# kubernetes-sigs/karpenter

Hardware: AMD Instinct MI355X
Metric: pods scheduled/sec (Solve()) (higher is better)
Workload: dtype int64

## Files before the change

karpenter_amd/csrc/fast_engine.h:

```cpp
#pragma once
#include <type_traits>
#include "kernels.h"
#include "pdq_emul.h"

namespace ks {

constexpr int kFastRows = 4;
constexpr uint32_t kFastFree = 0xFFFFFFFFu;
constexpr uint32_t kFastLastBit = 0x80000000u;
constexpr int kFastEnt = 1024;
constexpr int kFastPool = 256;
constexpr int kFastMaxPareto = 16;
constexpr int kFastMaxVar = 12;
constexpr uint64_t kFastExtBit = 1ull << 63;
constexpr int kFastVarBits = 56;

struct FastClaim { uint64_t vmask; int32_t req[4]; };
template <int R> struct FastRec { uint64_t vmask; int32_t req[4]; uint64_t acc[R]; };
struct FastSlot { uint64_t cvmask; uint64_t dmask; int32_t size[4]; uint32_t tmplok; uint32_t kdef; };
struct FastEnt { uint64_t vmask; int32_t cap[4]; uint32_t info; uint32_t pad; };

struct FastPlan {
  int total_bytes, cap;
  int off_state, off_key, off_ord, off_snap, off_ent, off_pool, off_slot, off_misc, off_hot;
  int global_state;
  int rows;
  int helper;
};

struct FastMisc {
  uint64_t tvmask[32];
  uint32_t tdef[32];
  uint64_t fmask[kFastMaxVar];
  uint8_t vkey[kFastMaxVar], voff[kFastMaxVar], vwidth[kFastMaxVar];
  uint16_t vword[kFastMaxVar];
  uint64_t its[kMaxItWords], rem[kMaxItWords], cand[kMaxItWords];
  uint64_t acc[kFastRows];
};

struct FastVar { int nv; uint8_t vkey[kFastMaxVar], voff[kFastMaxVar], vwidth[kFastMaxVar]; uint16_t vword[kFastMaxVar]; };

struct FastNodes {
  uint32_t n_left;
  uint32_t n_placed;
  uint32_t limit_hit;
  uint32_t variant;
  uint32_t bail;
  unsigned long long n_ref;
  unsigned long long n_tests;
};

struct FastWork {
  FastVar* var;
  FastSlot* cls;
  uint32_t* c_hostseq;
  uint16_t* c_ent;
  FastClaim* c_state;
  uint32_t* c_npods;
  uint64_t* ent_its;
  uint32_t* q_class;
  uint32_t* q_claim;
  uint32_t* q_cnt;
  uint16_t* o_key;
  uint16_t* o_ord;
  uint16_t* o_snap;
  uint64_t* c_rec;
  uint32_t* cls_first;
  uint32_t* cls_last;
  uint32_t* max_active;
  FastNodes* nodes;
  uint32_t* nd_pod;
  const uint64_t* nd_dead0;
  FastPlan plan;
  int enabled;
};

typedef uint64_t __attribute__((may_alias)) u64_alias;
template <class T>
KS_FN T lds_get(const KS_LDS T* p) {
  static_assert(sizeof(T) % 8 == 0, "lds_get: 8-byte multiples");
  T out;
  u64_alias* o = (u64_alias*)&out;
  const KS_LDS u64_alias* s = (const KS_LDS u64_alias*)p;
#pragma unroll
  for (int i = 0; i < (int)(sizeof(T) / 8); ++i) o[i] = s[i];
  return out;
}
template <class T>
KS_FN void lds_put(KS_LDS T* p, const T& v) {
  static_assert(sizeof(T) % 8 == 0, "lds_put: 8-byte multiples");
  const u64_alias* o = (const u64_alias*)&v;
  KS_LDS u64_alias* s = (KS_LDS u64_alias*)p;
#pragma unroll
  for (int i = 0; i < (int)(sizeof(T) / 8); ++i) s[i] = o[i];
}

// ... 143 lines not shown
KS_FN uint32_t fast_umin_s(uint32_t a, uint32_t b) {
#if KS_DEVICE
  uint32_t r;
  asm("s_min_u32 %0, %1, %2" : "=s"(r) : "s"(a), "s"(b) : "scc");
  return r;
#else
  return a < b ? a : b;
#endif
}
KS_FN bool fast_sampled(int n, int p) {
  const unsigned q = (unsigned)n >> 2, u = (unsigned)p;
  return u - (q - 1) <= 2u || u - (2 * q - 1) <= 2u || u - (3 * q - 1) <= 2u;
}

struct FastMail {
  uint32_t word[2];
  uint32_t done;
  uint32_t gen;
  uint32_t quit;
  int32_t miss_x[2];
  uint32_t helper;
  uint32_t simd[4];
};
#if KS_DEVICE
KS_FN uint32_t mail_load(const KS_LDS uint32_t* p) { return *(const volatile KS_LDS uint32_t*)p; }
KS_FN void mail_store(KS_LDS uint32_t* p, uint32_t v) { *(volatile KS_LDS uint32_t*)p = v; }
#else
KS_FN uint32_t mail_load(const uint32_t* p) { return *p; }
KS_FN void mail_store(uint32_t* p, uint32_t v) { *p = v; }
#endif

struct FastHot {
  alignas(16) FastMail mail;
  int base, bi, bn, n, np, max_steps, steps, status;
  int pend_a, pend_x, pend_new, ev_arg;
  uint32_t pend_mv;
  int rf_x;
  int rf_x2;
  unsigned long long n_steps, n_tests, n_ref, hot_cycles;
  unsigned long long tsec[8];
  unsigned long long hw[4];
  const uint32_t* q_class; const volatile int* cancel; uint32_t* q_claim; uint32_t* q_cnt;
  uint32_t cur[kFastRows][64];
  uint32_t scls[kFastRows][64];
  uint32_t bcls[64], oclaim[64], ocnt[64], nxt_cls[64];
};

template <class W, int GS, int R>
struct FastCold {
  const ProblemView* Pk;
  const Workspace* Sk;
  const FastWork* Fk;
  typedef typename FastMem<GS, R>::o16 o16;
  ClaimOrder<W, o16, false> order;
  typename FastMem<GS, R>::s16 snap;
  typename FastMem<GS, R>::States cst;
  KS_LDS FastEnt* ent;
  KS_LDS int32_t* pool;
  KS_LDS FastSlot* aslot;
  KS_LDS FastMisc* Mp;
  KS_LDS FastHot* hs;
  int n_claims = 0, nv = 0, n_ent = 0, n_pool = 0, n_evict = 0;
  uint32_t host_seq = 0, active_templates = 0;
  int bail_code = 0;
  int lo_ = 0, hi_ = -1;
  unsigned long long n_ref_extra = 0, n_cold_tests = 0;

  KS_DEV void init(const ProblemView* p, const Workspace* s, const FastWork* f, char* lds) {
    Pk = p; Sk = s; Fk = f;
    const FastPlan& pl = f->plan;
    Mp = (KS_LDS FastMisc*)(lds + pl.off_misc);
    hs = (KS_LDS FastHot*)(lds + pl.off_hot);
    if constexpr (GS >= 1) cst.p = (FastRec<R>*)f->c_rec; else cst.p = (KS_LDS FastRec<R>*)(lds + pl.off_state);
    typedef typename FastMem<GS, R>::s16 s16;
    if constexpr (GS >= 2) { order.key = (o16)f->o_key; order.ord = (o16)f->o_ord; }
    else { order.key = (o16)(lds + pl.off_key); order.ord = (o16)(lds + pl.off_ord); }
    if constexpr (GS >= 1) snap = (s16)f->o_snap; else snap = (s16)(lds + pl.off_snap);
    order.pos = nullptr;
    ent = (KS_LDS FastEnt*)(lds + pl.off_ent);
    pool = (KS_LDS int32_t*)(lds + pl.off_pool);
    aslot = (KS_LDS FastSlot*)(lds + pl.off_slot);
  }

  KS_COLD int create_entry(uint64_t vm) {
    vm = W::uniform(vm);
    const ProblemView& P = *Pk; const Workspace& S = *Sk; const FastWork& F = *Fk;
    const int t = (int)(vm >> 56);
    const int iw = P.it_words, n_its = P.n_its, nr = P.n_res;
    const Dict& d = P.dict;
    const ProblemView& Pv = P;
    KS_LDS FastMisc& Mm = *Mp;
    const uint64_t* tits = S.t_its + (size_t)t * iw;
    KS_LDS uint64_t* its = Mp->its;
    const int nvv = nv;
    W::for_n(iw, [&](int w) {
      uint64_t acc = tits[w];
      for (int j = 0; j < nvv; ++j) {
        const int k = Mm.vkey[j];
        if (!((Pv.it_keys >> k) & 1u)) continue;
        if ((vm >> (Mm.voff[j] + Mm.vwidth[j])) & 1) continue;
        uint64_t field = (vm >> Mm.voff[j]) & (Mm.fmask[j] >> Mm.voff[j]);
        uint64_t r = Pv.key_undef[(size_t)k * iw + w];
        const size_t base = (size_t)Mm.vword[j] * 64;
        while (field) { const int b = ctz64(field); field &= field - 1; r |= Pv.kv_has[(base + b) * iw + w]; }
        acc &= r;
      }
      its[w] = acc;
    });
    uint32_t zones = (1u << P.n_zones) - 1, cts = (1u << P.n_cts) - 1;
    {
      const uint64_t* tm = P.tmpl_reqs.mask + (size_t)t * d.req_words;
      const uint32_t tdef = Mp->tdef[t];
      if (d.key_zone >= 0 && ((tdef >> d.key_zone) & 1u)) zones &= (uint32_t)tm[d.key_word_off[d.key_zone]];
      if (d.key_ct >= 0 && ((tdef >> d.key_ct) & 1u)) cts &= (uint32_t)tm[d.key_word_off[d.key_ct]];
      for (int j = 0; j < nv; ++j) {
        const uint32_t field = (uint32_t)((vm >> Mp->voff[j]) & (Mp->fmask[j] >> Mp->voff[j]));
        if (Mp->vkey[j] == d.key_zone) zones &= field;
        if (Mp->vkey[j] == d.key_ct) cts &= field;
      }
    }
    uint64_t cells = 0;
    for (uint32_t z = zones; z; z &= z - 1) cells |= (uint64_t)cts << (__builtin_ctz(z) * 4);
    for (int j = 0; j < iw; ++j) {
      const uint64_t in = its[j];
      const uint64_t okm = in ? W::ballot([&](int l) { const int it = j * 64 + l; return it < n_its && ((in >> l) & 1) && (Pv.it_off_avail[it] & cells) != 0; }) : 0ull;
      W::store(&its[j], okm);
    }
    W::sync();
    if (n_ent * 5 >= kFastEnt * 4) return -1;
    uint32_t h = fast_hash(vm);
    while (ent[h].info & 1u) h = (h + 1) & (kFastEnt - 1);
    uint64_t* eits = F.ent_its + (size_t)h * iw;
    W::for_n(iw, [&](int w) { eits[w] = its[w]; });
    KS_LDS uint64_t* rem = Mp->rem; KS_LDS uint64_t* cand = Mp->cand;
    W::for_n(iw, [&](int w) { rem[w] = its[w]; });
    int count = 0;
    const int poff = n_pool;
    int32_t f0 = -1, f1 = -1, f2 = -1, f3 = -1;
    const int64_t* eff = eff_alloc(P, t);
    for (;;) {
      const uint64_t any = W::reduce_or(iw, [&](int w) { return (uint64_t)rem[w]; });
      if (!any) break;
      W::for_n(iw, [&](int w) { cand[w] = rem[w]; });
      int64_t v0 = 0x3FFFFFFF, v1 = 0x3FFFFFFF, v2 = 0x3FFFFFFF, v3 = 0x3FFFFFFF;
      for (int r = 0; r < nr; ++r) {
        const int64_t* al = eff + (size_t)r * n_its;
        const int64_t mx = W::reduce_max_i64(iw * 64, [&](int it) { return (it < n_its && ((cand[it >> 6] >> (it & 63)) & 1)) ? al[it] : INT64_MIN; });
        if (r == 0) v0 = mx; else if (r == 1) v1 = mx; else if (r == 2) v2 = mx; else v3 = mx;
        for (int j = 0; j < iw; ++j) {
          const uint64_t in = cand[j];
          const uint64_t eq = in ? W::ballot([&](int l) { const int it = j * 64 + l; return it < n_its && ((in >> l) & 1) && al[it] == mx; }) : 0ull;
          W::store(&cand[j], eq);
        }
        W::sync();
      }
      if (count == 0) { f0 = (int32_t)v0; f1 = (int32_t)v1; f2 = (int32_t)v2; f3 = (int32_t)v3; }
      else {
        if (count > kFastMaxPareto || n_pool >= kFastPool) return -1;
        if (W::leader()) { pool[n_pool * 4 + 0] = (int32_t)v0; pool[n_pool * 4 + 1] = (int32_t)v1; pool[n_pool * 4 + 2] = (int32_t)v2; pool[n_pool * 4 + 3] = (int32_t)v3; }
        n_pool++;
      }
      count++;
      for (int j = 0; j < iw; ++j) {
        const uint64_t in = rem[j];
        const uint64_t dom = in ? W::ballot([&](int l) {
          const int it = j * 64 + l;
          if (it >= n_its || !((in >> l) & 1)) return false;
          bool le = eff[it] <= v0;
          if (nr > 1) le = le && eff[(size_t)n_its + it] <= v1;
          if (nr > 2) le = le && eff[(size_t)2 * n_its + it] <= v2;
          if (nr > 3) le = le && eff[(size_t)3 * n_its + it] <= v3;
          return le;
        }) : 0ull;
        W::store(&rem[j], in & ~dom);
      }
      W::sync();
    }
    if (W::leader()) {
      FastEnt e;
      e.vmask = count > 1 ? (vm | kFastExtBit) : vm; e.cap[0] = f0; e.cap[1] = f1; e.cap[2] = f2; e.cap[3] = f3;
      e.info = 1u | ((uint32_t)(count > 1 ? count - 1 : 0) << 8) | ((uint32_t)poff << 16);
      e.pad = 0;
      lds_put(&ent[h], e);
    }
    n_ent++;
    W::sync();
    return (int)h;
  }

  KS_COLD int setup(bool topo = false) {
    const ProblemView& P = *Pk; const Workspace& S = *Sk; const FastWork& F = *Fk;
    const Dict& d = P.dict;
    const int nk = d.n_keys, iw = P.it_words, nr = P.n_res, n_its = P.n_its, nc = P.n_classes, T = P.n_templates;
    const ProblemView& Pv = P;
    if (!(topo ? P.plain_topo : (P.plain || (F.nodes && P.plain_nodes))) || P.n_rows != P.n_pods || nr > 4 || T > 32 || iw > kMaxItWords) return 1;
    if (W::reduce_or(T, [&](int t) { return (uint64_t)(Pv.tmpl_reqs.complement[t] | (Pv.tmpl_reqs.has_gte ? Pv.tmpl_reqs.has_gte[t] : 0) | (Pv.tmpl_reqs.has_lte ? Pv.tmpl_reqs.has_lte[t] : 0)); })) return 3;
    if (W::reduce_or(nc, [&](int c) { return (uint64_t)Pv.cls_reqs.complement[c]; })) return 4;
    uint32_t vk = (uint32_t)W::reduce_or(nc, [&](int c) { return (uint64_t)Pv.cls_reqs.defined[c]; });
    if (topo) vk |= (uint32_t)W::reduce_or(P.topo.n_groups, [&](int g) { return Pv.topo.key[g] >= 0 ? (uint64_t)1 << Pv.topo.key[g] : (uint64_t)0; });
    if (d.key_hostname >= 0 && ((vk >> d.key_hostname) & 1u)) return 5;
    if (d.key_it >= 0 && ((vk >> d.key_it) & 1u)) return 5;
    int bits = 0;
    nv = 0;
    for (int k = 0; k < nk; ++k) {
      if (!((vk >> k) & 1u)) continue;
      if (d.key_word_off[k + 1] - d.key_word_off[k] != 1 || nv >= kFastMaxVar) return 6;
      const uint64_t valid = d.value_valid[d.key_word_off[k]];
      const int width = valid ? 64 - __builtin_clzll(valid) : 1;
      if (bits + width + 1 > kFastVarBits) return 6;
      if (W::leader()) {
        Mp->vkey[nv] = (uint8_t)k; Mp->voff[nv] = (uint8_t)bits; Mp->vwidth[nv] = (uint8_t)width; Mp->vword[nv] = (uint16_t)d.key_word_off[k];
        Mp->fmask[nv] = ((1ull << width) - 1) << bits;
      }
      bits += width + 1;
      nv++;
    }
    W::sync();
    if (W::leader()) {
      FastVar fv;
      fv.nv = nv;
      for (int j = 0; j < kFastMaxVar; ++j) { fv.vkey[j] = Mp->vkey[j]; fv.voff[j] = Mp->voff[j]; fv.vwidth[j] = Mp->vwidth[j]; fv.vword[j] = Mp->vword[j]; }
      *F.var = fv;
    }
    W::sync();
    if (W::reduce_or(nr * n_its, [&](int i) { const int64_t a = Pv.it_alloc[i]; return (uint64_t)((a >= (1ll << 30) || a <= -(1ll << 30)) ? 1 : 0); })) return 7;
    for (int t = 0; t < T; ++t) {
      if (!((P.tmpl_ov >> t) & 1u)) continue;
      const int64_t* eff = eff_alloc(P, t);
      if (W::reduce_or(nr * n_its, [&](int i) { const int64_t a = eff[i]; return (uint64_t)((a >= (1ll << 30) || a <= -(1ll << 30)) ? 1 : 0); })) return 7;
    }
    if (W::reduce_or(nr * nc, [&](int i) { const int64_t a = Pv.cls_requests[i]; return (uint64_t)((a >= (1ll << 30) || a < 0) ? 1 : 0); })) return 7;
    KS_LDS FastMisc& Mm = *Mp;
    const int nvv = nv;
    W::for_n(T, [&](int t) {
      const uint64_t* tm = Pv.tmpl_reqs.mask + (size_t)t * d.req_words;
      const uint32_t tdef = Pv.tmpl_reqs.defined[t];
      uint64_t vm = (uint64_t)t << 56;
      for (int j = 0; j < nvv; ++j) {
        if ((tdef >> Mm.vkey[j]) & 1u) vm |= (tm[Mm.vword[j]] << Mm.voff[j]) & Mm.fmask[j];
        else vm |= Mm.fmask[j] | (1ull << (Mm.voff[j] + Mm.vwidth[j]));
      }
      Mm.tvmask[t] = vm; Mm.tdef[t] = tdef;
    });
    active_templates = 0;
    for (int t = 0; t < T; ++t) {
      const uint64_t* tm = P.tmpl_reqs.mask + (size_t)t * d.req_words;
      const uint32_t tdef = Mp->tdef[t];
      uint64_t* tits = S.t_its + (size_t)t * iw;
      const uint64_t* tin = P.tmpl_its + (size_t)t * iw;
      W::for_n(iw, [&](int w) {
        uint64_t acc = tin[w] & Pv.it_alloc_ok[w];
        for (int k = 0; k < nk; ++k) {
          if (!((tdef >> k) & 1u)) continue;
          const uint32_t w0 = d.key_word_off[k], w1 = d.key_word_off[k + 1];
          if (k == d.key_it) { acc &= tm[w0 + w]; continue; }
          if (!((Pv.it_keys >> k) & 1u)) continue;
          uint64_t r = Pv.key_undef[(size_t)k * iw + w];
          for (uint32_t x = w0; x < w1; ++x) for (uint64_t b = tm[x]; b; b &= b - 1) r |= Pv.kv_has[((size_t)x * 64 + ctz64(b)) * iw + w];
          acc &= r;
        }
        tits[w] = acc;
      });
      uint32_t zones = (1u << P.n_zones) - 1, cts = (1u << P.n_cts) - 1;
      if (d.key_zone >= 0 && ((tdef >> d.key_zone) & 1u)) zones &= (uint32_t)tm[d.key_word_off[d.key_zone]];
      if (d.key_ct >= 0 && ((tdef >> d.key_ct) & 1u)) cts &= (uint32_t)tm[d.key_word_off[d.key_ct]];
      uint64_t cells = 0;
      for (uint32_t z = zones; z; z &= z - 1) cells |= (uint64_t)cts << (__builtin_ctz(z) * 4);
      uint64_t any = 0;
      for (int j = 0; j < iw; ++j) {
        const uint64_t in = tits[j];
        const uint64_t okm = in ? W::ballot([&](int l) { const int it = j * 64 + l; return it < n_its && ((in >> l) & 1) && (Pv.it_off_avail[it] & cells) != 0; }) : 0ull;
// ... 270 lines not shown
        }
        if (excluded) { bail_code = 24; return 0; }
      }
      host_seq++;
      n_ref_extra++;
      if (!((cs.tmplok >> t) & 1u)) continue;
      const uint64_t m = Mp->tvmask[t] & cs.cvmask;
      if (!fast_fields_ok(m, cs.dmask)) continue;
      FastEnt e;
      int eh = fast_lookup(ent, m, e);
      if (eh < 0) { eh = create_entry(m); if (eh < 0) { bail_code = 25; return 0; } e = lds_get(&ent[eh]); }
      const int32_t zero[4] = {0, 0, 0, 0};
      if (!fast_fits(pool, e, zero, cs.size)) continue;
      if (n_claims >= S.max_claims) { bail_code = -1; return 0; }
      if (n_claims >= cap) { bail_code = 26; return 0; }
      const int c = n_claims++;
      FastClaim ns;
      ns.vmask = m;
      for (int q = 0; q < 4; ++q) ns.req[q] = cs.size[q];
      if (W::leader()) {
        cst.put_state((uint32_t)c, ns);
        F.c_hostseq[c] = host_seq;
        order.key[n] = 1; order.ord[n] = (uint16_t)c;
      }
      W::sync();
      for (int j = 0; j < R; ++j) {
        const uint64_t aw = row_accepts(ns, j);
        if (bail_code) return 0;
        if (W::leader()) { cst.put_acc((uint32_t)c, j, aw); Mp->acc[j] = aw; }
      }
      W::sync();
      if (lm) {
        int64_t* rem = S.t_remaining + (size_t)t * (nr + 1);
        const int64_t* eff = eff_alloc(P, t);
        const uint64_t* eits = F.ent_its + (size_t)eh * iw;
        const ProblemView& Pv = P;
        const int n_its = P.n_its;
        for (int q = 0; q < nr; ++q) if ((lm >> q) & 1) {
          const int64_t mx = W::reduce_max_i64(n_its, [&](int it) {
            if (!((eits[it >> 6] >> (it & 63)) & 1)) return INT64_MIN;
            for (int z = 0; z < nr; ++z) if (eff[(size_t)z * n_its + it] < (int64_t)cs.size[z]) return INT64_MIN;
            return Pv.it_cap[(size_t)q * n_its + it];
          });
          W::store(&rem[q], rem[q] - mx);
        }
        W::sync();
      }
      return 1;
    }
    bail_code = 27;
    return 0;
  }

  KS_COLD void finish(int status, int n, unsigned long long steps, unsigned long long n_steps, unsigned long long n_tests, unsigned long long n_ref, const unsigned long long* tc) {
    const Workspace& S = *Sk; const FastWork& F = *Fk;
    if (status != 3 && status != 1) {
      uint32_t* go = S.o_ord;
      const o16 oo = order.ord; const o16 ok_ = order.key;
      FastClaim* gs = F.c_state; uint32_t* gn = F.c_npods; uint16_t* ge = F.c_ent;
      const typename FastMem<GS, R>::States ls = cst;
      const KS_LDS FastEnt* en = ent;
      W::for_n(n, [&](int i) { const uint32_t c = oo[i]; go[i] = c; gn[c] = ok_[i]; });
      W::for_n(n, [&](int c) {
        const FastClaim st = ls.state((uint32_t)c);
        FastEnt e;
        gs[c] = st;
        ge[c] = (uint16_t)fast_lookup(en, st.vmask, e);
      });
      W::store(S.n_claims_out, n_claims);
    }
    FastNodes nd{};
    if (F.nodes) nd = *F.nodes;
    if (status == 0 && nd.limit_hit) status = 2;
    if (status) W::store(S.status_out, status);
    Counters c{};
    c.bin_evaluations = n_tests + n_cold_tests + nd.n_tests; c.full_evaluations = n_steps; c.queue_pops = steps + nd.n_placed; c.sorts = steps; c.slow_sorts = order.slow_sorts;
    c.column_resets = (unsigned long long)n_evict; c.ref_bin_evaluations = n_ref + n_ref_extra + nd.n_ref;
    c.cycles[20] = (unsigned long long)(bail_code > 0 ? bail_code : 0);
    if (tc) for (int i = 0; i < 16; ++i) c.cycles[i] = tc[i];
#ifdef KSOLVE_PHASE_TIMERS
    for (int i = 0; i < 4; ++i) c.cycles[16 + i] = hs->hw[i];
    c.cycles[18] = (hs->hw[2] << 32) | (unsigned long long)(hs->mail.simd[0] | (hs->mail.simd[1] << 8) | (hs->mail.simd[2] << 16) | (hs->mail.simd[3] << 24));
#endif
    if (F.nodes) c.cycles[19] = (unsigned long long)nd.variant;
    if (W::leader()) *S.counters = c;
    W::sync();
  }
};

template <int GS, int R>
struct FastHotCtx {
  typename FastMem<GS, R>::o16 okey, oord; typename FastMem<GS, R>::States cst; KS_LDS FastEnt* ent; KS_LDS int32_t* pool;
  KS_LDS FastSlot* aslot; KS_LDS FastHot* hs;
};
enum { FEV_DONE = 0, FEV_REFRESH = 1, FEV_SLOT = 2, FEV_SLOWSORT = 3, FEV_PLACE = 4, FEV_NEWCLAIM = 5, FEV_COUNT = 6, FEV_SLOW = 7, FEV_CONT = 8, FEV_DEAD = 9 };

template <int R>
struct FastHelperK {
  LaneVar<uint32_t> tok[R];
  LaneVar<uint64_t> cvm[R], dm[R], gd[R];
  LaneVar<int32_t> z0[R], z1[R], z2[R], z3[R];
  uint32_t gen = 0xFFFFFFFFu, miss = 0;
};
template <class W, int R>
KS_FN void fast_helper_consts(FastHelperK<R>& k, const KS_LDS FastSlot* aslot, const KS_LDS FastHot* hs) {
  W::each([&](int l) {
#pragma unroll
    for (int j = 0; j < R; ++j) {
      const FastSlot s = lds_get(&aslot[j * 64 + l]);
      k.cvm[j].at(l) = s.cvmask; k.dm[j].at(l) = s.dmask; k.gd[j].at(l) = (s.dmask << 1) & ~s.dmask;
      k.z0[j].at(l) = s.size[0]; k.z1[j].at(l) = s.size[1]; k.z2[j].at(l) = s.size[2]; k.z3[j].at(l) = s.size[3];
      k.tok[j].at(l) = hs->scls[j][l] == kFastFree ? 0u : s.tmplok;
    }
  });
}
template <class W, int GS, int R>
KS_FN void fast_helper_serve(FastHelperK<R>& k, FastHotCtx<GS, R> cx, uint32_t s_, uint32_t w_) {
  KS_LDS FastHot* const hs = cx.hs;
  KS_LDS FastMail* const mail = &hs->mail;
  W::order();
  const uint32_t gen = (uint32_t)fast_uniform((int)mail->gen);
  if (gen != k.gen) { fast_helper_consts<W, R>(k, cx.aslot, hs); k.gen = gen; k.miss = 0; }
  const uint32_t x = (uint32_t)fast_uniform((int)(w_ & 0xFFFFu));
  const FastClaim st = cx.cst.state(x);
  const uint64_t vmask = W::uniform(st.vmask);
  const int32_t req[4] = {fast_uniform(st.req[0]), fast_uniform(st.req[1]), fast_uniform(st.req[2]), fast_uniform(st.req[3])};
  const uint32_t tbit = 1u << (uint32_t)(vmask >> 56);
  LaneVar<uint64_t> mlv[R], evm[R];
  LaneVar<int32_t> c0[R], c1[R], c2[R], c3[R];
  W::each([&](int l) {
#pragma unroll
    for (int j = 0; j < R; ++j) {
      const uint64_t m = vmask & k.cvm[j].at(l);
      const FastEnt e = ent_live(&cx.ent[fast_hash(m)]);
      mlv[j].at(l) = m; evm[j].at(l) = e.vmask;
      c0[j].at(l) = e.cap[0]; c1[j].at(l) = e.cap[1]; c2[j].at(l) = e.cap[2]; c3[j].at(l) = e.cap[3];
    }
  });
  uint64_t accw[R];
  bool miss = false;
#pragma unroll
  for (int j = 0; j < R; ++j) {
    const uint64_t tokm = W::ballot([&](int l) { return (k.tok[j].at(l) & tbit) != 0; });
    const uint64_t fldm = W::ballot([&](int l) { return (((mlv[j].at(l) & k.dm[j].at(l)) + k.dm[j].at(l)) & k.gd[j].at(l)) == k.gd[j].at(l); });
    const uint64_t simm = W::ballot([&](int l) { return evm[j].at(l) == mlv[j].at(l); });
    const uint64_t f0 = W::ballot([&](int l) { return k.z0[j].at(l) <= c0[j].at(l) - req[0]; });
    const uint64_t f1 = W::ballot([&](int l) { return k.z1[j].at(l) <= c1[j].at(l) - req[1]; });
    const uint64_t f2 = W::ballot([&](int l) { return k.z2[j].at(l) <= c2[j].at(l) - req[2]; });
    const uint64_t f3 = W::ballot([&](int l) { return k.z3[j].at(l) <= c3[j].at(l) - req[3]; });
    const uint64_t basem = tokm & fldm, fitm = f0 & f1 & f2 & f3;
    uint64_t accm = basem & simm & fitm;
    const uint64_t oddm = basem & ~simm;
    if (KS_UNLIKELY(oddm != 0)) {
      uint64_t ok2 = 0, missm = 0;
      W::ballot2([&](int l) {
        if (!((oddm >> l) & 1)) return 0;
        FastEnt e;
        if (fast_lookup(cx.ent, mlv[j].at(l), e) < 0) return 2;
        const int32_t sz[4] = {k.z0[j].at(l), k.z1[j].at(l), k.z2[j].at(l), k.z3[j].at(l)};
        return fast_fits(cx.pool, e, req, sz) ? 1 : 0;
      }, ok2, missm);
      accm |= ok2;
      if (missm) miss = true;
    }
    accw[j] = accm;
  }
// ... 694 lines not shown
        const uint64_t f3 = W::ballot([&](int l) { return z3[j].at(l) <= c3[j].at(l) - ns.req[3]; });
        const uint64_t basem = tokm & fldm, fitm = f0 & f1 & f2 & f3;
        uint64_t accm = basem & simm & fitm;
        const uint64_t oddm = basem & ~simm;
        if (KS_UNLIKELY(oddm != 0)) {
          uint64_t ok2 = 0, missm = 0;
          W::ballot2([&](int l) {
            if (!((oddm >> l) & 1)) return 0;
            FastEnt e;
            if (fast_lookup(ent, mlv[j].at(l), e) < 0) return 2;
            const int32_t sz[4] = {z0[j].at(l), z1[j].at(l), z2[j].at(l), z3[j].at(l)};
            return fast_fits(pool, e, ns.req, sz) ? 1 : 0;
          }, ok2, missm);
          accm |= ok2;
          if (missm) { rf = x; bfx = bi + 1; }
        }
        accw[j] = accm;
      }
      W::each([&](int l) {
        if (l == fo_) {
          FastRec<R> mine;
          mine.vmask = nmv.at(l); mine.req[0] = n0v.at(l); mine.req[1] = n1v.at(l); mine.req[2] = n2v.at(l); mine.req[3] = n3v.at(l);
#pragma unroll
          for (int j = 0; j < R; ++j) mine.acc[j] = accw[j];
          cst.put_rec(xw.at(l), mine);
        }
      });
      if constexpr (FastMem<GS, R>::kStateHbm) W::hbm_sync(); else W::order();
      gather();
      bi++; steps++;
    }
    if (bi < bf || bf < bn || rf >= 0) break;
    if (bn > 0) {
      const int dn = bn, b0 = base;
      W::each([&](int l) { if (l < dn) { gqclaim[b0 + l] = oclaim.at(l); gqcnt[b0 + l] = ocnt.at(l); } });
    }
    const int nbase = bn > 0 ? base + 64 : base;
    if (nbase >= np || (polled && (nbase & 1023) == 0)) break;
    base = nbase;
    bn = np - base < 64 ? np - base : 64;
    bi = 0;
    const int nb = base + 64;
    W::each([&](int l) { bcls.at(l) = nxt_cls.at(l); });
    W::each([&](int l) { if (nb + l < np) nxt_cls.at(l) = gqcls[nb + l]; });
  }
  int rf2 = -1;
  if constexpr (HP) {
    const uint32_t dw = wait_for(seq);
    if (KS_UNLIKELY((dw & 1u) != 0)) {
      rf = fast_uniform((int)mail->miss_x[0]); rf2 = fast_uniform((int)mail->miss_x[1]);
      if (rf < 0) { rf = rf2; rf2 = -1; }
      W::order();
      if (W::leader()) { mail->miss_x[0] = -1; mail->miss_x[1] = -1; mail_store(&mail->done, seq << 1); }
      W::order();
    }
    if (KS_UNLIKELY(dead)) return FEV_DEAD;
#ifdef KSOLVE_PHASE_TIMERS
    if (W::leader()) { hs->hw[0] += hw0; hs->hw[1] += hw1; hs->hw[2] += hw2; hs->hw[3] += hw3; }
#endif
  }
  if (bi != bi_in || base != base_in) {
    if (W::leader()) { hs->base = base; hs->bi = bi; hs->bn = bn; hs->steps = steps; hs->n_ref = n_ref; hs->rf_x = rf; hs->rf_x2 = rf2; hs->n_steps += 4 * n_ext; }
    W::each([&](int l) {
#pragma unroll
      for (int j = 0; j < R; ++j) { hs->cur[j][l] = cur[j].at(l); hs->scls[j][l] = scls[j].at(l); }
      hs->nxt_cls[l] = nxt_cls.at(l); hs->bcls[l] = bcls.at(l); hs->oclaim[l] = oclaim.at(l); hs->ocnt[l] = ocnt.at(l);
    });
    W::sync();
  }
  return FEV_SLOW;
}

template <class W, int GS = 0, int R = 1, bool HP = false>
struct FastEngine {
  FastCold<W, GS, R> cold;
  KS_LDS FastHot* hs;
  KS_DEV FastEngine(const ProblemView* p, const Workspace* s, const FastWork* f, char* lds) { cold.init(p, s, f, lds); hs = cold.hs; }

  KS_DEV void solve() {
    KS_LDS FastHot* const h = fast_uniform(hs);
    W::each([&](int l) { for (int j = 0; j < kFastRows; ++j) { h->cur[j][l] = 0; h->scls[j][l] = kFastFree; } });
    W::sync();
    {
      const int why = (int)W::uniform((uint64_t)(uint32_t)cold.setup());
      if (why) { cold.bail_code = why; cold.finish(3, 0, 0, 0, 0, 0, nullptr); return; }
    }
    const FastNodes* const nds = fast_uniform(cold.Fk->nodes);
    if (nds && fast_uniform((int)nds->bail) != 0) { cold.bail_code = fast_uniform((int)nds->bail); cold.finish(3, 0, 0, 0, 0, 0, nullptr); return; }
    const int np = nds ? fast_uniform((int)nds->n_left) : fast_uniform(cold.Pk->n_pods);
    if (W::leader()) {
      h->base = 0; h->bi = 0; h->bn = 0; h->n = 0; h->np = np; h->steps = 0; h->status = 0;
      const long long ms_ = cold.Sk->max_steps;
      h->max_steps = ms_ < 0 ? -1 : (nds || ms_ > 0x7FFFFFFF) ? 0x7FFFFFFF : (int)ms_;
      h->pend_a = -1; h->pend_x = 0; h->pend_mv = 0; h->pend_new = 0; h->ev_arg = 0; h->rf_x = -1; h->rf_x2 = -1;
      h->n_steps = 0; h->n_tests = 0; h->n_ref = 0; h->hot_cycles = 0;
      for (int i = 0; i < 8; ++i) h->tsec[i] = 0;
      for (int i = 0; i < 4; ++i) h->hw[i] = 0;
      h->q_class = cold.Fk->q_class; h->cancel = cold.Sk->cancel_flag;
      h->q_claim = cold.Fk->q_claim; h->q_cnt = cold.Fk->q_cnt;
    }
    {
      const uint32_t* qc = cold.Fk->q_class;
      W::each([&](int l) { h->nxt_cls[l] = l < np ? qc[l] : 0; h->bcls[l] = 0; h->oclaim[l] = 0; h->ocnt[l] = 0; });
    }
    W::sync();
    FastHotCtx<GS, R> cx;
    cx.okey = cold.order.key; cx.oord = cold.order.ord; cx.cst = cold.cst; cx.ent = cold.ent; cx.pool = cold.pool;
    cx.aslot = cold.aslot; cx.hs = hs;
    unsigned long long tev[8] = {0, 0, 0, 0, 0, 0, 0, 0}, nev[8] = {0, 0, 0, 0, 0, 0, 0, 0};
    unsigned long long t_fast = 0, n_fast = 0, t_slow = 0, n_slow = 0;
    const unsigned long long t_begin = W::clock();
    const bool use_fast = fast_uniform(h->max_steps) < 0;
    for (;;) {
      const unsigned long long tf0 = W::clock();
      const bool place_now = use_fast && fast_uniform(h->pend_new) != 0 && fast_uniform(h->bi) < fast_uniform(h->bn) && fast_uniform(h->status) == 0;
      int ev = place_now ? (int)FEV_PLACE : use_fast ? fast_uniform(fast_hot_run<W, GS, R, HP>(cx)) : (int)FEV_SLOW;
      t_fast += W::clock() - tf0; n_fast++;
      if (HP && ev == FEV_DEAD) { cold.bail_code = 28; cold.finish(3, 0, 0, 0, 0, 0, nullptr); return; }
      if (use_fast && fast_uniform(h->rf_x) >= 0) {
        const int rx = fast_uniform(h->rf_x), rx2 = HP ? fast_uniform(h->rf_x2) : -1;
        if (W::leader()) { h->rf_x = -1; h->rf_x2 = -1; }
        W::sync();
        if (fast_uniform(cold.refresh_claim(rx)) < 0) { cold.bail_code = 21; cold.finish(3, 0, 0, 0, 0, 0, nullptr); return; }
        if (rx2 >= 0 && fast_uniform(cold.refresh_claim(rx2)) < 0) { cold.bail_code = 21; cold.finish(3, 0, 0, 0, 0, 0, nullptr); return; }
        continue;
      }
      if (ev == FEV_SLOW) { const unsigned long long ts0 = W::clock(); ev = fast_uniform(fast_slow_run<W, GS, R>(cx, use_fast ? 1 : 0x7FFFFFFF)); t_slow += W::clock() - ts0; n_slow++; }
      if (ev == FEV_CONT) continue;
      if (ev == FEV_DONE) break;
      const unsigned long long te0 = W::clock();
      if (ev == FEV_REFRESH) {
        if (fast_uniform(cold.refresh_claim(fast_uniform(h->ev_arg))) < 0) { cold.bail_code = 21; cold.finish(3, 0, 0, 0, 0, 0, nullptr); return; }
      } else if (ev == FEV_SLOT) {
        if (fast_uniform(cold.new_slot(fast_uniform(h->ev_arg))) < 0) { cold.finish(3, 0, 0, 0, 0, 0, nullptr); return; }
      } else if (ev == FEV_SLOWSORT || ev == FEV_PLACE) {
        const int n = fast_uniform(h->n);
        int b = -1;
        if (ev == FEV_SLOWSORT) cold.slow_sort(n, fast_uniform(h->ev_arg), 0);
        else b = fast_uniform(cold.place_new_claim(n));
        if (b == -1) {
          const int lo = fast_uniform(cold.lo_), hi = fast_uniform(cold.hi_);
          if (hi >= lo) W::each([&](int l) { for (int j = 0; j < R; ++j) { const uint32_t r = h->cur[j][l]; if (r > (uint32_t)lo && r <= (uint32_t)hi) h->cur[j][l] = (uint32_t)lo; } });
        } else {
          const KS_LDS uint64_t* acc = cold.Mp->acc;
          W::each([&](int l) { for (int j = 0; j < R; ++j) { const uint32_t r = h->cur[j][l]; if (r > (uint32_t)b) h->cur[j][l] = ((acc[j] >> l) & 1) ? (uint32_t)b : r + 1; } });
        }
        if (W::leader()) { h->pend_a = -1; h->pend_new = 0; }
        W::sync();
      } else if (ev == FEV_NEWCLAIM) {
        const int n = fast_uniform(h->n), bi = fast_uniform(h->bi);
        const int made = fast_uniform(cold.new_claim(fast_uniform(h->ev_arg), bi, n));
        if (!made) { cold.finish(fast_uniform(cold.bail_code) < 0 ? 1 : 3, 0, (unsigned long long)fast_uniform(h->steps), 0, 0, 0, nullptr); return; }
        if (W::leader()) { h->oclaim[bi] = (uint32_t)n; h->ocnt[bi] = 0; h->n = n + 1; h->pend_new = 1; h->pend_a = 0x7FFFFFFF; h->bi = bi + 1; }
        W::sync();
      } else { cold.bail_code = 22; cold.finish(3, 0, 0, 0, 0, 0, nullptr); return; }
      if (ev >= 1 && ev <= 5) { tev[ev] += W::clock() - te0; nev[ev]++; }
    }
    unsigned long long tc[16] = {h->hot_cycles, tev[1], tev[2], tev[3], tev[4], tev[5], W::clock() - t_begin, nev[3] + (nev[4] << 20) + (nev[1] << 40),
                                 t_fast, n_fast, t_slow, n_slow, nev[1], nev[2], nev[3] + (nev[4] << 32), nev[5]};
    const unsigned long long steps = (unsigned long long)fast_uniform(h->steps);
    cold.finish(fast_uniform(h->status), fast_uniform(h->n), steps, h->n_steps + steps, steps * (unsigned long long)(64 * R), h->n_ref, tc);
  }
};

struct FastQueueArgs {
  const uint32_t* sorted; const uint32_t* row_class;
  uint32_t* q_class; uint32_t* q_claim; uint32_t* q_cnt;
// ... 78 lines not shown
```

karpenter_amd/csrc/wave.h:

```cpp
#pragma once
#include <stdint.h>

#if defined(__HIPCC__) && !defined(KSOLVE_HOST_EMULATION)
#define KS_DEVICE 1
#define KS_FN __host__ __device__ __forceinline__
#define KS_DEV __device__ __forceinline__
#define KS_LDS __attribute__((address_space(3)))
#define KS_GLOBAL __attribute__((address_space(1)))
#else
#define KS_DEVICE 0
#define KS_FN inline
#define KS_DEV inline
#define KS_LDS
#define KS_GLOBAL
#endif

namespace ks {

#if KS_DEVICE

struct Wave {
  KS_DEV static int lane() { return (int)(threadIdx.x & 63); }
  KS_DEV static uint64_t uniform(uint64_t v) {
    const uint32_t lo = (uint32_t)__builtin_amdgcn_readfirstlane((int)(uint32_t)v), hi = (uint32_t)__builtin_amdgcn_readfirstlane((int)(uint32_t)(v >> 32));
// ... 34 lines not shown
  KS_DEV static void for_n(int n, F f) {
    for (int i = lane(); i < n; i += 64) f(i);
    sync();
  }
  template <class F>
  KS_DEV static int find_first(int lo, int hi, F pred) {
    for (int base = lo; base < hi; base += 64) {
      int i = base + lane();
      uint64_t m = __builtin_amdgcn_ballot_w64(i < hi && pred(i));
      if (m) return base + __builtin_ctzll(m);
    }
    return hi;
  }
  template <class F>
  KS_DEV static int find_last(int lo, int hi, F pred) {
    for (int top = hi; top > lo; top -= 64) {
      int i = top - 64 + lane();
      uint64_t m = __builtin_amdgcn_ballot_w64(i >= lo && pred(i));
      if (m) return top - 64 + (63 - __builtin_clzll(m));
    }
    return lo - 1;
  }
  template <class F>
  KS_DEV static int find_first8(int lo, int hi, F pred) {
    for (int base = lo; base < hi; base += 512) {
      int r[8];
#pragma unroll
      for (int j = 0; j < 8; ++j) { const int i = base + j * 64 + lane(); r[j] = (i < hi && pred(i)) ? 1 : 0; }
#pragma unroll
      for (int j = 0; j < 8; ++j) { const uint64_t m = __ballot(r[j]); if (m) return base + j * 64 + __builtin_ctzll(m); }
    }
    return hi;
  }
  template <class F>
  KS_DEV static int find_last8(int lo, int hi, F pred) {
    for (int top = hi; top > lo; top -= 512) {
      int r[8];
#pragma unroll
      for (int j = 0; j < 8; ++j) { const int i = top - (j + 1) * 64 + lane(); r[j] = (i >= lo && pred(i)) ? 1 : 0; }
#pragma unroll
      for (int j = 0; j < 8; ++j) { const uint64_t m = __ballot(r[j]); if (m) return top - (j + 1) * 64 + (63 - __builtin_clzll(m)); }
    }
    return lo - 1;
  }
  template <class D, class S>
  KS_DEV static void copy8(D dst, S src, int n) {
    for (int base = 0; base < n; base += 512) {
      decltype(src[0] + 0) v[8];
#pragma unroll
      for (int j = 0; j < 8; ++j) { const int i = base + j * 64 + lane(); if (i < n) v[j] = src[i]; }
#pragma unroll
      for (int j = 0; j < 8; ++j) { const int i = base + j * 64 + lane(); if (i < n) dst[i] = (decltype(dst[0] + 0))v[j]; }
    }
    sync();
  }
  template <class F>
  KS_DEV static uint64_t reduce_min(int n, F f) {
    uint64_t v = ~0ull;
    for (int i = lane(); i < n; i += 64) { uint64_t x = f(i); v = x < v ? x : v; }
    for (int off = 32; off > 0; off >>= 1) {
      uint64_t o = __shfl_xor(v, off, 64);
      v = o < v ? o : v;
    }
    return uniform(v);
  }
  template <class F>
  KS_DEV static int64_t reduce_max_i64(int n, F f) {
    int64_t v = INT64_MIN;
    for (int i = lane(); i < n; i += 64) { int64_t x = f(i); v = x > v ? x : v; }
    for (int off = 32; off > 0; off >>= 1) {
      int64_t o = __shfl_xor(v, off, 64);
      v = o > v ? o : v;
    }
    return (int64_t)uniform((uint64_t)v);
  }
  template <class F>
  KS_DEV static int64_t lanes_max_i64(F f) {
    int64_t v = f(lane());
    for (int off = 32; off > 0; off >>= 1) {
      int64_t o = __shfl_xor(v, off, 64);
      v = o > v ? o : v;
    }
    return (int64_t)uniform((uint64_t)v);
  }
  template <class F>
  KS_DEV static uint64_t reduce_or(int n, F f) {
    uint64_t v = 0;
    for (int i = lane(); i < n; i += 64) v |= f(i);
    for (int off = 32; off > 0; off >>= 1) v |= __shfl_xor(v, off, 64);
    return uniform(v);
  }
  template <class T, class V>
  KS_DEV static void store(T* p, V v) {
    if (lane() == 0) *p = (T)v;
  }
  template <class T, class V>
  KS_DEV static void store(KS_LDS T* p, V v) {
    if (lane() == 0) *p = (T)v;
  }
  KS_DEV static bool leader() { return lane() == 0; }
  template <class F>
  KS_DEV static void each(F f) { f(lane()); }
  KS_DEV static int poll_flag(const volatile int* p) { return __hip_atomic_load(p, __ATOMIC_RELAXED, __HIP_MEMORY_SCOPE_SYSTEM); }
#ifdef KSOLVE_PHASE_TIMERS
  KS_DEV static unsigned long long clock() { return __builtin_readcyclecounter(); }
#else
  KS_DEV static unsigned long long clock() { return 0ull; }
#endif
  KS_DEV static uint32_t min_u32(uint32_t v) {
    int x = (int)v;
#define KS_DPP_MIN(ctrl, row_mask) { int o = __builtin_amdgcn_update_dpp(-1, x, ctrl, row_mask, 0xf, false); x = ((uint32_t)o < (uint32_t)x) ? o : x; }
    KS_DPP_MIN(0xB1, 0xf)
    KS_DPP_MIN(0x4E, 0xf)
    KS_DPP_MIN(0x124, 0xf)
    KS_DPP_MIN(0x128, 0xf)
    KS_DPP_MIN(0x142, 0xa)
    KS_DPP_MIN(0x143, 0xc)
#undef KS_DPP_MIN
    return (uint32_t)__builtin_amdgcn_readlane(x, 63);
  }
  template <class F>
  KS_DEV static uint32_t argmin_u32(F f, int* lane_out) {
    uint32_t mine = f(lane());
    uint32_t m = min_u32(mine);
    uint64_t who = __builtin_amdgcn_ballot_w64(mine == m);
    *lane_out = m == 0xFFFFFFFFu ? -1 : (int)__builtin_ctzll(who);
    return m;
  }
};

#else

#ifdef KS_EMU_REVERSE_LANES
#define KS_LANES(l) for (int l = 63; l >= 0; --l)
#else
#define KS_LANES(l) for (int l = 0; l < 64; ++l)
#endif

struct Wave {
  static int lane() { return 0; }
  static uint64_t uniform(uint64_t v) { return v; }
  static void sync() {}
  static void order() {}
  static void sched_fence() {}
  static void hbm_sync() {}
  template <class F>
  static uint64_t ballot(F f) {
    uint64_t m = 0;
    KS_LANES(l) if (f(l)) m |= 1ull << l;
    return m;
  }
  template <class F>
  static void ballot4(F f, uint64_t& m0, uint64_t& m1, uint64_t& m2, uint64_t& m3) {
    m0 = m1 = m2 = m3 = 0;
    KS_LANES(l) { const int v = f(l); if (v & 1) m0 |= 1ull << l; if (v & 2) m1 |= 1ull << l; if (v & 4) m2 |= 1ull << l; if (v & 8) m3 |= 1ull << l; }
  }
  template <class F>
  static void ballot2(F f, uint64_t& m0, uint64_t& m1) {
    m0 = m1 = 0;
    KS_LANES(l) { const int v = f(l); if (v & 1) m0 |= 1ull << l; if (v & 2) m1 |= 1ull << l; }
  }
  template <class F, class G>
  static void ballots8(int n, F f, G g) {
    for (int j = 0; j < n; ++j) { uint64_t m = 0; KS_LANES(l) if (f(l, j)) m |= 1ull << l; g(j, m); }
  }
  template <class F>
  static void for_n(int n, F f) {
    for (int base = 0; base < n; base += 64) KS_LANES(l) if (base + l < n) f(base + l);
  }
  template <class F>
  static int find_first(int lo, int hi, F pred) { for (int i = lo; i < hi; ++i) if (pred(i)) return i; return hi; }
  template <class F>
  static int find_last(int lo, int hi, F pred) { for (int i = hi - 1; i >= lo; --i) if (pred(i)) return i; return lo - 1; }
  template <class F>
  static uint64_t reduce_min(int n, F f) { uint64_t v = ~0ull; for_n(n, [&](int i) { uint64_t x = f(i); if (x < v) v = x; }); return v; }
  template <class F>
  static int find_first8(int lo, int hi, F pred) { return find_first(lo, hi, pred); }
  template <class F>
  static int find_last8(int lo, int hi, F pred) { return find_last(lo, hi, pred); }
  template <class D, class S>
  static void copy8(D dst, S src, int n) { for (int i = 0; i < n; ++i) dst[i] = src[i]; }
  template <class F>
  static int64_t reduce_max_i64(int n, F f) { int64_t v = INT64_MIN; for_n(n, [&](int i) { int64_t x = f(i); if (x > v) v = x; }); return v; }
  template <class F>
  static int64_t lanes_max_i64(F f) { int64_t v = INT64_MIN; KS_LANES(l) { int64_t x = f(l); if (x > v) v = x; } return v; }
  template <class F>
  static uint64_t reduce_or(int n, F f) { uint64_t v = 0; for_n(n, [&](int i) { v |= f(i); }); return v; }
  template <class T, class V>
  static void store(T* p, V v) { *p = (T)v; }
  static bool leader() { return true; }
  template <class F>
  static void each(F f) { KS_LANES(l) f(l); }
#if defined(KSOLVE_PHASE_TIMERS) && defined(__x86_64__)
  static unsigned long long clock() { return __builtin_ia32_rdtsc(); }
#else
  static unsigned long long clock() { return 0; }
#endif
  static int poll_flag(const volatile int* p) { return __atomic_load_n(p, __ATOMIC_RELAXED); }
  template <class F>
  static uint32_t argmin_u32(F f, int* lane_out) {
    uint32_t m = 0xFFFFFFFFu; int who = -1;
    KS_LANES(l) { uint32_t x = f(l); if (x < m || (x == m && who >= 0 && l < who)) { m = x; who = l; } }
    *lane_out = who;
    return m;
  }
};

#endif

struct LaneVec64 {
#if KS_DEVICE
  uint64_t v = 0;
  KS_DEV void set(int lane, uint64_t x) {
    uint32_t lo = (uint32_t)v, hi = (uint32_t)(v >> 32);
    const uint32_t xl = (uint32_t)x, xh = (uint32_t)(x >> 32);
    uint32_t m0_saved;
    asm volatile("s_mov_b32 %2, m0\n\ts_mov_b32 m0, %4\n\tv_writelane_b32 %0, %3, m0\n\tv_writelane_b32 %1, %5, m0\n\ts_mov_b32 m0, %2"
                 : "+v"(lo), "+v"(hi), "=&s"(m0_saved) : "s"(xl), "s"(lane), "s"(xh));
    v = (uint64_t)lo | ((uint64_t)hi << 32);
  }
  KS_DEV uint64_t get(int) const { return v; }
#else
  uint64_t v[64] = {};
  void set(int lane, uint64_t x) { v[lane] = x; }
  uint64_t get(int l) const { return v[l]; }
#endif
};

template <class T>
struct LaneVar {
#if KS_DEVICE
  T v;
  KS_DEV T& at(int) { return v; }
  KS_DEV T v_of(int) const { return v; }
  KS_DEV void set(int lane, T x) {
    static_assert(sizeof(T) == 4, "LaneVar::set: 32-bit values");
    uint32_t w = __builtin_bit_cast(uint32_t, v), m0_saved;
    const uint32_t xs = (uint32_t)__builtin_amdgcn_readfirstlane((int)__builtin_bit_cast(uint32_t, x));
    lane = __builtin_amdgcn_readfirstlane(lane);
    asm volatile("s_mov_b32 %1, m0\n\ts_mov_b32 m0, %3\n\tv_writelane_b32 %0, %2, m0\n\ts_mov_b32 m0, %1" : "+v"(w), "=&s"(m0_saved) : "s"(xs), "s"(lane));
    v = __builtin_bit_cast(T, w);
  }
  KS_DEV T shuffle(int, int src) const {
    static_assert(sizeof(T) == 4 || sizeof(T) == 8, "LaneVar::shuffle: 32- or 64-bit values");
    if constexpr (sizeof(T) == 4) {
      const int x = __builtin_amdgcn_ds_bpermute(src << 2, __builtin_bit_cast(int, v));
      return __builtin_bit_cast(T, x);
    } else {
      const uint64_t u = __builtin_bit_cast(uint64_t, v);
      const uint32_t lo = (uint32_t)__builtin_amdgcn_ds_bpermute(src << 2, (int)(uint32_t)u);
      const uint32_t hi = (uint32_t)__builtin_amdgcn_ds_bpermute(src << 2, (int)(uint32_t)(u >> 32));
      return __builtin_bit_cast(T, (uint64_t)lo | ((uint64_t)hi << 32));
    }
  }
  KS_DEV T bcast(int lane) const {
    static_assert(sizeof(T) == 4 || sizeof(T) == 8, "LaneVar: 32- or 64-bit values");
    if constexpr (sizeof(T) == 4) {
      const int x = __builtin_amdgcn_readlane(__builtin_bit_cast(int, v), lane);
      return __builtin_bit_cast(T, x);
    } else {
      const uint64_t u = __builtin_bit_cast(uint64_t, v);
      const uint32_t lo = (uint32_t)__builtin_amdgcn_readlane((int)(uint32_t)u, lane);
      const uint32_t hi = (uint32_t)__builtin_amdgcn_readlane((int)(uint32_t)(u >> 32), lane);
      return __builtin_bit_cast(T, (uint64_t)lo | ((uint64_t)hi << 32));
    }
  }
#else
  T v[64];
// ... 13 lines not shown
```

Before: 1.546 million.

## Add register-resident create_entry path for narrow instance-type word counts

Adds a create_entry_regs path, used when it_words is at most 8. It keeps the instance-type filter words and the per-resource allocations in lane registers instead of LDS arrays. Requirement filtering is spread across lane slots and combined with shuffle ANDs, and the Pareto extraction uses packed per-lane bitmasks with a new DPP-based 32-bit max reduction. Optional phase timers are also added. The aim is to cut LDS round-trips, syncs and per-word ballots in cold entry creation. The cost is much higher register pressure and a truncation of int64 allocations to int32.

```diff
diff --git a/karpenter_amd/csrc/fast_engine.h b/karpenter_amd/csrc/fast_engine.h
--- a/karpenter_amd/csrc/fast_engine.h
+++ b/karpenter_amd/csrc/fast_engine.h
@@ -12,6 +12,7 @@
 constexpr int kFastPool = 256;
 constexpr int kFastMaxPareto = 16;
 constexpr int kFastMaxVar = 12;
+constexpr int kFastRegWords = 8;
 constexpr uint64_t kFastExtBit = 1ull << 63;
 constexpr int kFastVarBits = 56;
 
@@ -321,8 +322,182 @@
     aslot = (KS_LDS FastSlot*)(lds + pl.off_slot);
   }
 
-  KS_COLD int create_entry(uint64_t vm) {
+#ifdef KSOLVE_PHASE_TIMERS
+  unsigned long long tm_setup = 0, tm_filter = 0, tm_pareto = 0;
+#define KS_COLD_TIME(acc, t0) ((acc) += W::clock() - (t0))
+#else
+#define KS_COLD_TIME(acc, t0) ((void)(t0))
+#endif
+
+  KS_DEV int create_entry(uint64_t vm) {
+    const int iw = fast_uniform(Pk->it_words);
+    return (iw >= 1 && iw <= kFastRegWords) ? create_entry_regs(vm) : create_entry_wide(vm);
+  }
+
+  KS_COLD int create_entry_regs(uint64_t vm) {
+    static_assert(kFastRegWords == 8, "lane = 8 slot + word below; W::ballots8");
     vm = W::uniform(vm);
+    const unsigned long long tc0 = W::clock();
+    const ProblemView& P = *Pk; const Workspace& S = *Sk; const FastWork& F = *Fk;
+    const int t = (int)(vm >> 56);
+    const int iw = P.it_words, n_its = P.n_its, nr = P.n_res;
+    const Dict& d = P.dict;
+    const ProblemView& Pv = P;
+    KS_LDS FastMisc& Mm = *Mp;
+    const uint64_t* tits = S.t_its + (size_t)t * iw;
+    const int nvv = nv;
+    LaneVar<uint64_t> part, other;
+    W::each([&](int l) {
+      const int w = l % kFastRegWords, s = l / kFastRegWords;
+      uint64_t acc = ~0ull;
+      if (w < iw) {
+        if (s == 0) acc = tits[w];
+        int seen = 0;
+        for (int j = 0; j < nvv; ++j) {
+          const int k = Mm.vkey[j];
+          if (!((Pv.it_keys >> k) & 1u)) continue;
+          if ((vm >> (Mm.voff[j] + Mm.vwidth[j])) & 1) continue;
+          if ((seen++ % (64 / kFastRegWords)) != s) continue;
+          uint64_t field = (vm >> Mm.voff[j]) & (Mm.fmask[j] >> Mm.voff[j]);
+          const uint64_t* kv = Pv.kv_has + (size_t)Mm.vword[j] * 64 * iw + w;
+          uint64_t r = Pv.key_undef[(size_t)k * iw + w];
+          while (field) {
+            uint64_t x0 = 0, x1 = 0, x2 = 0, x3 = 0;
+            { x0 = kv[(size_t)ctz64(field) * iw]; field &= field - 1; }
+            if (field) { x1 = kv[(size_t)ctz64(field) * iw]; field &= field - 1; }
+            if (field) { x2 = kv[(size_t)ctz64(field) * iw]; field &= field - 1; }
+            if (field) { x3 = kv[(size_t)ctz64(field) * iw]; field &= field - 1; }
+            r |= (x0 | x1) | (x2 | x3);
+          }
+          acc &= r;
+        }
+      }
+      part.at(l) = acc;
+    });
+    for (int off = kFastRegWords; off < 64; off <<= 1) {
+      W::each([&](int l) { other.at(l) = part.shuffle(l, l ^ off); });
+      W::each([&](int l) { part.at(l) &= other.at(l); });
+    }
+    uint64_t cw[kFastRegWords];
+#pragma unroll
+    for (int j = 0; j < kFastRegWords; ++j) cw[j] = j < iw ? W::uniform(part.bcast(j)) : 0ull;
+    uint32_t zones = (1u << P.n_zones) - 1, cts = (1u << P.n_cts) - 1;
+    {
+      const uint64_t* tm = P.tmpl_reqs.mask + (size_t)t * d.req_words;
+      const uint32_t tdef = Mp->tdef[t];
+      if (d.key_zone >= 0 && ((tdef >> d.key_zone) & 1u)) zones &= (uint32_t)tm[d.key_word_off[d.key_zone]];
+      if (d.key_ct >= 0 && ((tdef >> d.key_ct) & 1u)) cts &= (uint32_t)tm[d.key_word_off[d.key_ct]];
+      for (int j = 0; j < nv; ++j) {
+        const uint32_t field = (uint32_t)((vm >> Mp->voff[j]) & (Mp->fmask[j] >> Mp->voff[j]));
+        if (Mp->vkey[j] == d.key_zone) zones &= field;
+        if (Mp->vkey[j] == d.key_ct) cts &= field;
+      }
+    }
+    uint64_t cells = 0;
+    for (uint32_t z = zones; z; z &= z - 1) cells |= (uint64_t)cts << (__builtin_ctz(z) * 4);
+    uint64_t itw[kFastRegWords] = {0, 0, 0, 0, 0, 0, 0, 0};
+    W::ballots8(iw, [&](int l, int j) {
+      const int it = j * 64 + l;
+      const uint64_t av = Pv.it_off_avail[it < n_its ? it : n_its - 1];
+      return (int)(it < n_its) & (int)((cw[j] >> l) & 1) & (int)((av & cells) != 0);
+    }, [&](int j, uint64_t m) { itw[j] = m; });
+    if (n_ent * 5 >= kFastEnt * 4) return -1;
+    uint32_t h = fast_hash(vm);
+    while (ent[h].info & 1u) h = (h + 1) & (kFastEnt - 1);
+    uint64_t* eits = F.ent_its + (size_t)h * iw;
+    W::each([&](int l) {
+      uint64_t v = 0;
+#pragma unroll
+      for (int j = 0; j < kFastRegWords; ++j) if (l == j) v = itw[j];
+      if (l < iw) eits[l] = v;
+    });
+    W::sync();
+    KS_COLD_TIME(tm_filter, tc0);
+    const unsigned long long tc1 = W::clock();
+    const int64_t* eff = eff_alloc(P, t);
+    LaneVar<int32_t> a[4][kFastRegWords];
+    LaneVar<uint32_t> remb, candb;
+    W::each([&](int l) {
+      uint32_t rb = 0;
+#pragma unroll
+      for (int j = 0; j < kFastRegWords; ++j) rb |= (uint32_t)((itw[j] >> l) & 1) << j;
+      remb.at(l) = rb;
+      int64_t x[4][kFastRegWords];
+#pragma unroll
+      for (int r = 0; r < 4; ++r) {
+#pragma unroll
+        for (int j = 0; j < kFastRegWords; ++j) {
+          const int it = j * 64 + l;
+          x[r][j] = (r < nr && j < iw) ? eff[(size_t)r * n_its + (it < n_its ? it : n_its - 1)] : 0;
+        }
+      }
+#pragma unroll
+      for (int r = 0; r < 4; ++r) {
+#pragma unroll
+        for (int j = 0; j < kFastRegWords; ++j) a[r][j].at(l) = ((rb >> j) & 1) ? (int32_t)x[r][j] : INT32_MIN;
+      }
+    });
+    int count = 0;
+    const int poff = n_pool;
+    int32_t f0 = -1, f1 = -1, f2 = -1, f3 = -1;
+    for (;;) {
+      if (!W::ballot([&](int l) { return remb.v_of(l) != 0; })) break;
+      W::each([&](int l) { candb.at(l) = remb.at(l); });
+      int32_t v[4] = {0x3FFFFFFF, 0x3FFFFFFF, 0x3FFFFFFF, 0x3FFFFFFF};
+#pragma unroll
+      for (int r = 0; r < 4; ++r) {
+        if (r >= nr) continue;
+        const int32_t mx = W::lanes_max_i32([&](int l) {
+          const uint32_t cb = candb.v_of(l);
+          int32_t m = INT32_MIN;
+#pragma unroll
+          for (int j = 0; j < kFastRegWords; ++j) { const int32_t y = ((cb >> j) & 1) ? a[r][j].v_of(l) : INT32_MIN; m = y > m ? y : m; }
+          return m;
+        });
+        v[r] = mx;
+        W::each([&](int l) {
+          uint32_t eq = 0;
+#pragma unroll
+          for (int j = 0; j < kFastRegWords; ++j) eq |= (uint32_t)(a[r][j].v_of(l) == mx) << j;
+          candb.at(l) &= eq;
+        });
+      }
+      if (count == 0) { f0 = v[0]; f1 = v[1]; f2 = v[2]; f3 = v[3]; }
+      else {
+        if (count > kFastMaxPareto || n_pool >= kFastPool) return -1;
+        if (W::leader()) { pool[n_pool * 4 + 0] = v[0]; pool[n_pool * 4 + 1] = v[1]; pool[n_pool * 4 + 2] = v[2]; pool[n_pool * 4 + 3] = v[3]; }
+        n_pool++;
+      }
+      count++;
+      W::each([&](int l) {
+        uint32_t dom = 0;
+#pragma unroll
+        for (int j = 0; j < kFastRegWords; ++j) {
+          bool le = a[0][j].v_of(l) <= v[0];
+          if (nr > 1) le = le & (a[1][j].v_of(l) <= v[1]);
+          if (nr > 2) le = le & (a[2][j].v_of(l) <= v[2]);
+          if (nr > 3) le = le & (a[3][j].v_of(l) <= v[3]);
+          dom |= (uint32_t)le << j;
+        }
+        remb.at(l) &= ~dom;
+      });
+    }
+    if (W::leader()) {
+      FastEnt e;
+      e.vmask = count > 1 ? (vm | kFastExtBit) : vm; e.cap[0] = f0; e.cap[1] = f1; e.cap[2] = f2; e.cap[3] = f3;
+      e.info = 1u | ((uint32_t)(count > 1 ? count - 1 : 0) << 8) | ((uint32_t)poff << 16);
+      e.pad = 0;
+      lds_put(&ent[h], e);
+    }
+    n_ent++;
+    W::sync();
+    KS_COLD_TIME(tm_pareto, tc1);
+    return (int)h;
+  }
+
+  KS_COLD int create_entry_wide(uint64_t vm) {
+    vm = W::uniform(vm);
+    const unsigned long long tc0 = W::clock();
     const ProblemView& P = *Pk; const Workspace& S = *Sk; const FastWork& F = *Fk;
     const int t = (int)(vm >> 56);
     const int iw = P.it_words, n_its = P.n_its, nr = P.n_res;
@@ -371,6 +546,8 @@
     while (ent[h].info & 1u) h = (h + 1) & (kFastEnt - 1);
     uint64_t* eits = F.ent_its + (size_t)h * iw;
     W::for_n(iw, [&](int w) { eits[w] = its[w]; });
+    KS_COLD_TIME(tm_filter, tc0);
+    const unsigned long long tc1 = W::clock();
     KS_LDS uint64_t* rem = Mp->rem; KS_LDS uint64_t* cand = Mp->cand;
     W::for_n(iw, [&](int w) { rem[w] = its[w]; });
     int count = 0;
@@ -424,8 +601,10 @@
     }
     n_ent++;
     W::sync();
+    KS_COLD_TIME(tm_pareto, tc1);
     return (int)h;
   }
+#undef KS_COLD_TIME
 
   KS_COLD int setup(bool topo = false) {
     const ProblemView& P = *Pk; const Workspace& S = *Sk; const FastWork& F = *Fk;
@@ -862,6 +1041,9 @@
     for (int i = 0; i < 4; ++i) c.cycles[16 + i] = hs->hw[i];
     c.cycles[18] = (hs->hw[2] << 32) | (unsigned long long)(hs->mail.simd[0] | (hs->mail.simd[1] << 8) | (hs->mail.simd[2] << 16) | (hs->mail.simd[3] << 24));
 #endif
+#ifdef KSOLVE_PHASE_TIMERS
+    if (!F.plan.helper) { c.cycles[16] = tm_setup; c.cycles[17] = tm_filter; c.cycles[18] = tm_pareto; }
+#endif
     if (F.nodes) c.cycles[19] = (unsigned long long)nd.variant;
     if (W::leader()) *S.counters = c;
     W::sync();
@@ -1722,7 +1904,13 @@
     W::each([&](int l) { for (int j = 0; j < kFastRows; ++j) { h->cur[j][l] = 0; h->scls[j][l] = kFastFree; } });
     W::sync();
     {
+      const unsigned long long ts0 = W::clock();
       const int why = (int)W::uniform((uint64_t)(uint32_t)cold.setup());
+#ifdef KSOLVE_PHASE_TIMERS
+      cold.tm_setup = W::clock() - ts0;
+#else
+      (void)ts0;
+#endif
       if (why) { cold.bail_code = why; cold.finish(3, 0, 0, 0, 0, 0, nullptr); return; }
     }
     const FastNodes* const nds = fast_uniform(cold.Fk->nodes);
diff --git a/karpenter_amd/csrc/wave.h b/karpenter_amd/csrc/wave.h
--- a/karpenter_amd/csrc/wave.h
+++ b/karpenter_amd/csrc/wave.h
@@ -140,6 +140,19 @@
       v = o > v ? o : v;
     }
     return (int64_t)uniform((uint64_t)v);
+  }
+  template <class F>
+  KS_DEV static int32_t lanes_max_i32(F f) {
+    int x = (int)f(lane());
+#define KS_DPP_MAX(ctrl, row_mask) { int o = __builtin_amdgcn_update_dpp(INT32_MIN, x, ctrl, row_mask, 0xf, false); x = o > x ? o : x; }
+    KS_DPP_MAX(0xB1, 0xf)
+    KS_DPP_MAX(0x4E, 0xf)
+    KS_DPP_MAX(0x124, 0xf)
+    KS_DPP_MAX(0x128, 0xf)
+    KS_DPP_MAX(0x142, 0xa)
+    KS_DPP_MAX(0x143, 0xc)
+#undef KS_DPP_MAX
+    return (int32_t)__builtin_amdgcn_readlane(x, 63);
   }
   template <class F>
   KS_DEV static uint64_t reduce_or(int n, F f) {
@@ -242,6 +255,8 @@
   static int64_t reduce_max_i64(int n, F f) { int64_t v = INT64_MIN; for_n(n, [&](int i) { int64_t x = f(i); if (x > v) v = x; }); return v; }
   template <class F>
   static int64_t lanes_max_i64(F f) { int64_t v = INT64_MIN; KS_LANES(l) { int64_t x = f(l); if (x > v) v = x; } return v; }
+  template <class F>
+  static int32_t lanes_max_i32(F f) { int32_t v = INT32_MIN; KS_LANES(l) { int32_t x = f(l); if (x > v) v = x; } return v; }
   template <class F>
   static uint64_t reduce_or(int n, F f) { uint64_t v = 0; for_n(n, [&](int i) { v |= f(i); }); return v; }
   template <class T, class V>
```

Result: no change. 1.544 million (-0.1%).
